# yubster4525/image_compression_2

Measured on AMD Instinct MI355X. Metric: images/sec encode+decode 256px, higher is better.
Workload: dtype f16 (synthesis) / split-bf16 (encoder); 1 GPU; batch=32 256x256 encode+8bit quantize+decode, SG3-T-256 generator; global_batch=32, per_gpu_batch=32, resolution=256, generator=stylegan3-t-256 (random init), encoder=HVAE_VGG_Encoder(img_resolution=1024), quantization_bits=8, parallelism=dp1 (batch-sharded, RCCL metric all_reduce)

## Files before the change

image_compression_2_amd/csrc/conv_common.h:

```cpp
#pragma once
#include "common.h"

namespace ic2 {

typedef __attribute__((ext_vector_type(8))) __bf16 bf16x8;
typedef __attribute__((ext_vector_type(8))) _Float16 f16x8;
typedef __attribute__((ext_vector_type(4))) float f32x4;

template <bool F16>
__device__ __forceinline__ f32x4 mfma32(bf16x8 a, bf16x8 b, f32x4 c) {
  if constexpr (F16)
    return __builtin_amdgcn_mfma_f32_16x16x32_f16(__builtin_bit_cast(f16x8, a), __builtin_bit_cast(f16x8, b), c, 0, 0, 0);
  else
    return __builtin_amdgcn_mfma_f32_16x16x32_bf16(a, b, c, 0, 0, 0);
}
__host__ __device__ inline bool is16(int dtype) { return dtype == IC2_BF16 || dtype == IC2_F16; }

struct IgemmArgs {
  const void* x;
  const void* w;
  void* y;
  const float* oscale;
  const float* bias;
  float* ws;
  int n, h, w_, cin_p, cout_p, cout_valid, kh, kw, pad, ho, wo;
  int M;
  int K;
  int nq;
  int tiles_o;
  int nblocks;
  int group;
  int korder;
  int o_base;
  int tile_base;
  int act;
  float slope, act_gain, clamp, out_mul;
  int out_layout, out_dtype;
  double* gn_part;
  int gn_groups, gn_c;
  const float* in_gn;
  float in_slope;
  int x_pix, x_hb32;
  int x_img, x_plane;
  int wx_twp, wx_th, wx_ns, wx_hp, wx_nh, wx_tx, wx_ty;
  int out_ieee;
};
__device__ __forceinline__ int ig_xb32(const IgemmArgs& a, int b) { return b >= a.x_hb32 ? b - a.x_hb32 : b; }
__device__ __forceinline__ uint32_t ig_halo_off(const IgemmArgs& a, int nn, int iy, int ix, int chunk) {
  return (uint32_t)((nn * a.x_img + (iy * a.w_ + ix) * a.x_pix) * 2 + (chunk >> 1) * a.x_plane + (chunk & 1) * 16);
}
inline void ig_set_input_layout(IgemmArgs& a, bool blocked) {
  if (blocked) a.x_pix = 16;
  a.x_img = blocked ? a.cin_p * a.h * a.w_ : a.x_pix * a.h * a.w_;
  a.x_plane = blocked ? a.h * a.w_ * 32 : 32;
}

__device__ __forceinline__ float4 ig_load_oscale(const IgemmArgs& a, int nn, int ob) {
  return a.oscale && ob < a.cout_p ? *reinterpret_cast<const float4*>(a.oscale + (int64_t)nn * a.cout_p + ob)
                                   : make_float4(1.f, 1.f, 1.f, 1.f);
}
__device__ __forceinline__ float4 ig_load_bias(const IgemmArgs& a, int ob) {
  return a.bias && ob < a.cout_p ? *reinterpret_cast<const float4*>(a.bias + ob) : make_float4(0.f, 0.f, 0.f, 0.f);
}
__device__ __forceinline__ void ig_preloads_done() { __builtin_amdgcn_s_waitcnt(0x0F70); }

__device__ __forceinline__ void ig_store4v(const IgemmArgs& a, int p, int nn, int pix, int ob, const float (&acc)[4],
                                           float4 sc, float4 bi, float (*vout)[4] = nullptr) {
  const float scv[4] = {sc.x, sc.y, sc.z, sc.w}, biv[4] = {bi.x, bi.y, bi.z, bi.w};
  float v[4];
#pragma unroll
  for (int r = 0; r < 4; ++r) {
    float t = acc[r] * scv[r] + biv[r];
    if (a.act) t = lrelu_gain_clamp(t, a.slope, a.act_gain, a.clamp);
    v[r] = t * a.out_mul;
  }
  if (vout != nullptr) {
#pragma unroll
    for (int r = 0; r < 4; ++r) (*vout)[r] = v[r];
  }
  if (a.out_layout != IC2_LAYOUT_NCHW) {
    const int64_t e = a.out_layout == IC2_LAYOUT_NHWC
                          ? (int64_t)p * a.cout_p + ob
                          : (((int64_t)nn * (a.cout_p >> 4) + (ob >> 4)) * ((int64_t)a.ho * a.wo) + pix) * 16 + (ob & 15);
    if (a.out_dtype == IC2_BF16) {
      uint2 pk;
      pk.x = (uint32_t)f2bf(v[0]) | ((uint32_t)f2bf(v[1]) << 16);
      pk.y = (uint32_t)f2bf(v[2]) | ((uint32_t)f2bf(v[3]) << 16);
      *reinterpret_cast<uint2*>(reinterpret_cast<bf16_t*>(a.y) + e) = pk;
    } else if (a.out_dtype == IC2_F16) {
      typedef _Float16 h2 __attribute__((ext_vector_type(2)));
      float s_[4];
#pragma unroll
      for (int r = 0; r < 4; ++r) s_[r] = a.out_ieee ? v[r] : __builtin_amdgcn_fmed3f(v[r], -65504.f, 65504.f);
      const h2 q0 = h2{(_Float16)s_[0], (_Float16)s_[1]}, q1 = h2{(_Float16)s_[2], (_Float16)s_[3]};
      if (vout != nullptr) {
        (*vout)[0] = (float)q0.x; (*vout)[1] = (float)q0.y; (*vout)[2] = (float)q1.x; (*vout)[3] = (float)q1.y;
      }
      uint2 pk;
      pk.x = __builtin_bit_cast(uint32_t, q0);
      pk.y = __builtin_bit_cast(uint32_t, q1);
      *reinterpret_cast<uint2*>(reinterpret_cast<uint16_t*>(a.y) + e) = pk;
    } else {
      *reinterpret_cast<float4*>(reinterpret_cast<float*>(a.y) + e) = make_float4(v[0], v[1], v[2], v[3]);
    }
  } else {
    float* yo = reinterpret_cast<float*>(a.y);
    const int hw = a.ho * a.wo;
#pragma unroll
    for (int r = 0; r < 4; ++r)
      if (ob + r < a.cout_valid) yo[((int64_t)nn * a.cout_valid + ob + r) * hw + pix] = v[r];
  }
}
__device__ __forceinline__ void ig_store4(const IgemmArgs& a, int p, int nn, int pix, int ob, const float (&acc)[4]) {
  ig_store4v(a, p, nn, pix, ob, acc, ig_load_oscale(a, nn, ob), ig_load_bias(a, ob));
}

__device__ __forceinline__ int xcd_remap(int b, int nblocks) {
  const int xcd = b & 7, loc = b >> 3;
  const int q8 = nblocks >> 3, r8 = nblocks & 7;
  return (xcd < r8 ? xcd * (q8 + 1) : r8 * (q8 + 1) + (xcd - r8) * q8) + loc;
}

template <int I, int J>
__device__ __forceinline__ void ig_epilogue(const IgemmArgs& a, const f32x4 (&acc)[I][J], int obase, int pbase, int fr,
                                            int fh) {
  const int hw = a.ho * a.wo;
  if (gridDim.y > 1) {
#pragma unroll
    for (int j = 0; j < J; ++j) {
      const int p = pbase + j * 16 + fr;
      if (p >= a.M) continue;
#pragma unroll
      for (int i = 0; i < I; ++i) {
        const int ob = obase + i * 16 + 4 * fh;
        if (ob < a.cout_p) *reinterpret_cast<f32x4*>(a.ws + ((int64_t)blockIdx.y * a.M + p) * a.cout_p + ob) = acc[i][j];
      }
    }
    return;
  }
  float4 bi[I];
#pragma unroll
  for (int i = 0; i < I; ++i) bi[i] = ig_load_bias(a, obase + i * 16 + 4 * fh);
#pragma unroll
  for (int j = 0; j < J; ++j) {
    const int p = pbase + j * 16 + fr;
    const int pc = p < a.M ? p : a.M - 1;
    const int nn = pc / hw;
    const int pix = pc - nn * hw;
    float4 sc[I];
#pragma unroll
    for (int i = 0; i < I; ++i) sc[i] = ig_load_oscale(a, nn, obase + i * 16 + 4 * fh);
    ig_preloads_done();
    if (p >= a.M) continue;
#pragma unroll
    for (int i = 0; i < I; ++i) {
      const int ob = obase + i * 16 + 4 * fh;
      if (ob >= a.cout_p) continue;
      const float v[4] = {acc[i][j][0], acc[i][j][1], acc[i][j][2], acc[i][j][3]};
      ig_store4v(a, p, nn, pix, ob, v, sc[i], bi[i]);
    }
  }
}

__device__ __forceinline__ void tile_coords(int logical, int tiles_o, int tiles_p, int group, int& o_tile,
                                            int& p_tile) {
  const int per = group * tiles_o;
  const int gi = logical / per;
  const int rem = logical - gi * per;
  const int gsz = min(group, tiles_p - gi * group);
  o_tile = rem / gsz;
  p_tile = gi * group + (rem - o_tile * gsz);
}

constexpr uint32_t kOob = 0x7ffffff0u;
constexpr int kRsrcWord3 = 0x00020000;

}
```

image_compression_2_amd/csrc/wino.hip:

```cpp
#include "conv_common.h"

namespace ic2 {

constexpr int WX_BO = 128, WX_NW = 8, WX_NS = 3;
constexpr int WX_SLAB = 4 * WX_BO * 64;
constexpr int WX_HROWS = 384, WX_HALO = WX_HROWS * 64;
constexpr int WX_HPW = WX_HROWS / 16 / WX_NW;
constexpr int WX_SLACK = 8 * 1024;
constexpr int WX_LDS = WX_NS * WX_SLAB + 2 * WX_HALO + WX_SLACK;
static_assert(WX_LDS <= 160 * 1024, "LDS");

typedef __attribute__((ext_vector_type(4))) uint32_t wx_u4;
__device__ __forceinline__ f16x8 wx_sub(f16x8 a, f16x8 b) {
  const wx_u4 x = __builtin_bit_cast(wx_u4, a), y = __builtin_bit_cast(wx_u4, b);
  wx_u4 r;
#pragma unroll
  for (int i = 0; i < 4; ++i) asm("v_pk_add_f16 %0, %1, %2 neg_lo:[0,1] neg_hi:[0,1]" : "=v"(r[i]) : "v"(x[i]), "v"(y[i]));
  return __builtin_bit_cast(f16x8, r);
}
__device__ __forceinline__ f16x8 wx_add(f16x8 a, f16x8 b) {
  const wx_u4 x = __builtin_bit_cast(wx_u4, a), y = __builtin_bit_cast(wx_u4, b);
  wx_u4 r;
#pragma unroll
  for (int i = 0; i < 4; ++i) asm("v_pk_add_f16 %0, %1, %2" : "=v"(r[i]) : "v"(x[i]), "v"(y[i]));
  return __builtin_bit_cast(f16x8, r);
}

__device__ __forceinline__ int wx_off(int row, int chunk) { return row * 64 + ((chunk ^ (((row >> 2) & 1) << 1)) << 4); }
__device__ __forceinline__ int wx_hoff(int line, int hp, int idx, int chunk) {
  return (line * hp + idx) * 64 + ((chunk ^ (((idx >> 2) & 1) << 1)) << 4);
}

#ifndef IC2_WX_ABL
#define IC2_WX_ABL 0
#endif
#ifndef IC2_WX_STAMP
#define IC2_WX_STAMP 0
#endif
#ifndef IC2_WX_SCHED
#define IC2_WX_SCHED 0
#endif
#ifndef IC2_WX_PRIO
#define IC2_WX_PRIO 0
#endif

__global__ void __launch_bounds__(512, 1) wino_fx_f16_kernel(IgemmArgs a) {
  __shared__ __attribute__((aligned(16))) char lds[WX_LDS];
  char* const wsl = lds;
  char* const hal = lds + WX_NS * WX_SLAB;
  const int tid = threadIdx.x;
  const int lane = tid & 63;
  const int wid = __builtin_amdgcn_readfirstlane(tid >> 6);
  const int half = wid >> 2;
  const int pg = wid & 3;
  const int fr = lane & 15, fh = lane >> 4;

  const int logical = xcd_remap(blockIdx.x, a.nblocks);
  const int per_group = a.group * (a.nblocks / a.tiles_o);
  const int gi = logical / per_group, grem = logical - gi * per_group;
  const int o_tile = gi * a.group + grem % a.group;
  int pt = grem / a.group;
  const int tx = pt % a.wx_tx;
  pt /= a.wx_tx;
  const int ty = pt % a.wx_ty;
  const int nn = pt / a.wx_ty;
  const int o0 = o_tile * WX_BO;
  const int twp = a.wx_twp, hp = a.wx_hp;
  const int oy0 = ty * a.wx_th, px0 = tx * twp;

  const char* __restrict__ xg = reinterpret_cast<const char*>(a.x);
  const char* __restrict__ ug = reinterpret_cast<const char*>(a.w);
  const int lrow = lane >> 2, pch = lane & 3;

  uint32_t w_off[2][2];
#pragma unroll
  for (int h = 0; h < 2; ++h)
#pragma unroll
    for (int k = 0; k < 2; ++k) {
      const int row = (wid + WX_NW * k) * 16 + lrow;
      const int nu = row >> 6, ol = h * 64 + (row & 63), o = o0 + ol;
      w_off[h][k] =
          o < a.cout_p ? (uint32_t)(((ol * 12 + nu) * a.cin_p) * 2 + ((pch ^ (((row >> 2) & 1) << 1)) << 4)) : kOob;
    }
  const char* const ug0 = ug + (int64_t)o0 * 12 * a.cin_p * 2;
  uint32_t h_off[WX_HPW];
#pragma unroll
  for (int k = 0; k < WX_HPW; ++k) {
    const int l = (wid + WX_NW * k) * 16 + lrow;
    const int line = l / hp, idx = l - line * hp;
    const int iy = oy0 - a.pad + (line >> 1), ix = 2 * px0 - a.pad + 2 * idx + (line & 1);
    const bool ok = l < a.wx_nh && (unsigned)iy < (unsigned)a.h && (unsigned)ix < (unsigned)a.w_;
    h_off[k] = ok ? ig_halo_off(a, nn, iy, ix, pch ^ (((idx >> 2) & 1) << 1)) : kOob;
  }
  int boff[2][3];
  const int ns = a.wx_ns;
#pragma unroll
  for (int jb = 0; jb < 2; ++jb) {
    const int b = pg * 2 + jb;
    const int rr = min(b / ns, a.wx_th - 1), t = (b % ns) * 16 + fr;
#pragma unroll
    for (int m = 0; m < 3; ++m) {
      const int j = half + m;
      boff[jb][m] = wx_hoff(rr * 2 + (j & 1), hp, t + (j >> 1), fh);
    }
  }
  const int ky_step = 2 * hp * 64;
  const int aoff = wx_off(fr, fh) + half * 2 * 64 * 64;
  const int CB = a.cin_p >> 5;
  const int x_cb = 2 * a.x_plane;

  auto issue_hs = [&](int cb, int j) {
    const __amdgpu_buffer_rsrc_t rs = __builtin_amdgcn_make_buffer_rsrc(
        (void*)(ug0 + ((int64_t)(4 * (j >> 1)) * a.cin_p + cb * 32) * 2), 0, cb < CB ? kOob : 0, kRsrcWord3);
    char* dst = wsl + j * (WX_SLAB / 2);
#pragma unroll
    for (int k = 0; k < 2; ++k)
      __builtin_amdgcn_raw_ptr_buffer_load_lds(
          rs, (__attribute__((address_space(3))) void*)(dst + (wid + WX_NW * k) * 1024), 16, w_off[j & 1][k], 0, 0, 0);
  };
  auto issue_hp = [&](int cb, int k) {
    const __amdgpu_buffer_rsrc_t rs =
        __builtin_amdgcn_make_buffer_rsrc((void*)(xg + (int64_t)cb * x_cb), 0, cb < CB ? kOob : 0, kRsrcWord3);
    __builtin_amdgcn_raw_ptr_buffer_load_lds(
        rs, (__attribute__((address_space(3))) void*)(hal + (cb & 1) * WX_HALO + (wid + WX_NW * k) * 1024), 16,
        h_off[k], 0, 0, 0);
  };

  f32x4 acc[2][8][2];
#pragma unroll
  for (int nl = 0; nl < 2; ++nl)
#pragma unroll
    for (int i = 0; i < 8; ++i)
#pragma unroll
      for (int jb = 0; jb < 2; ++jb) acc[nl][i][jb] = f32x4{0.f, 0.f, 0.f, 0.f};

  f16x8 d[2][3];
  f16x8 v[2][2];
  auto read_d = [&](const char* hl) {
#pragma unroll
    for (int jb = 0; jb < 2; ++jb)
#pragma unroll
      for (int m = 0; m < 3; ++m) d[jb][m] = *reinterpret_cast<const f16x8*>(hl + boff[jb][m]);
  };
  auto make_v = [&]() {
    if (half == 0) {
#pragma unroll
      for (int jb = 0; jb < 2; ++jb) {
        v[0][jb] = wx_sub(d[jb][0], d[jb][2]);
        v[1][jb] = wx_add(d[jb][1], d[jb][2]);
      }
    } else {
#pragma unroll
      for (int jb = 0; jb < 2; ++jb) {
        v[0][jb] = wx_sub(d[jb][1], d[jb][0]);
        v[1][jb] = wx_sub(d[jb][0], d[jb][2]);
      }
    }
  };

  issue_hp(0, 0);
  issue_hp(0, 1);
  issue_hp(0, 2);
#pragma unroll
  for (int j = 0; j < 5; ++j) issue_hs(0, j);
  issue_hp(1, 0);
  if constexpr (IC2_WX_SCHED == 2) {
    asm volatile("s_waitcnt vmcnt(5)" ::: "memory");
  } else {
    issue_hp(1, 1);
    asm volatile("s_waitcnt vmcnt(6)" ::: "memory");
  }
  __builtin_amdgcn_s_barrier();
  read_d(hal);
  bf16x8 af[2][4];
  auto read_a = [&](const char* wl, int nl) {
#pragma unroll
    for (int i = 0; i < 4; ++i) af[nl][i] = *reinterpret_cast<const bf16x8*>(wl + (nl * 64 + i * 16) * 64);
  };
  if (half == 1) __builtin_amdgcn_s_barrier();
  __builtin_amdgcn_sched_barrier(0);

  uint64_t st[7] = {0, 0, 0, 0, 0, 0, 0};
  uint64_t t_prev = 0, t_loop = 0;
  auto stamp = [&](int k) {
    if constexpr (IC2_WX_STAMP) {
      const uint64_t t = __builtin_amdgcn_s_memtime();
      st[k] += t - t_prev;
      t_prev = t;
    }
  };
  if constexpr (IC2_WX_STAMP) t_loop = t_prev = __builtin_amdgcn_s_memtime();
  for (int cb = 0; cb < CB; ++cb) {
    const char* hb_cur = hal + (cb & 1) * WX_HALO;
    const char* hb_nxt = hal + ((cb + 1) & 1) * WX_HALO;
#pragma unroll
    for (int j = 0; j < 6; ++j) {
      const int ky = j >> 1, hx = j & 1;
      const char* wl = wsl + j * (WX_SLAB / 2) + aoff;
      auto r_dma = [&]() {
        if (!(IC2_WX_ABL & 1) || cb == 0) issue_hs(cb + (j + 5) / 6, (j + 5) % 6);
        if constexpr (IC2_WX_SCHED == 2) {
          if (j == 0) issue_hp(cb + 1, 1);
          if (j == 1) issue_hp(cb + 1, 2);
          if (j == 5) issue_hp(cb + 2, 0);
        } else {
          if (j == 0) issue_hp(cb + 1, 2);
          if (j >= 4) issue_hp(cb + 2, j - 4);
        }
      };
      if constexpr (IC2_WX_PRIO == 2) __builtin_amdgcn_s_setprio(1);
      if constexpr (IC2_WX_SCHED >= 1) r_dma();
      if (hx == 0) make_v();
      read_a(wl, 0);
      read_a(wl, 1);
      if (hx == 1 && IC2_WX_SCHED < 2) {
        if constexpr (!(IC2_WX_ABL & 4)) read_d(ky < 2 ? hb_cur + (ky + 1) * ky_step : hb_nxt);
      }
      if constexpr (IC2_WX_STAMP) {
        __builtin_amdgcn_sched_barrier(0);
        stamp(0);
      }
      if constexpr (IC2_WX_SCHED == 0) r_dma();
      __builtin_amdgcn_sched_barrier(0);
      stamp(1);
      if constexpr (!(IC2_WX_ABL & 16)) {
        if constexpr (IC2_WX_SCHED == 2) {
          if (j == 1) asm volatile("s_waitcnt vmcnt(9)" ::: "memory");
          if (j == 0 || j == 2) asm volatile("s_waitcnt vmcnt(8)" ::: "memory");
          if (j == 3 || j == 5) asm volatile("s_waitcnt vmcnt(7)" ::: "memory");
          if (j == 4) asm volatile("s_waitcnt vmcnt(6)" ::: "memory");
        } else {
          if (j == 0) asm volatile("s_waitcnt vmcnt(9)" ::: "memory");
          if (j == 1 || j == 5) asm volatile("s_waitcnt vmcnt(8)" ::: "memory");
          if (j == 2 || j == 4) asm volatile("s_waitcnt vmcnt(7)" ::: "memory");
          if (j == 3) asm volatile("s_waitcnt vmcnt(6)" ::: "memory");
        }
      }
      stamp(2);
      if constexpr (!(IC2_WX_ABL & 2)) __builtin_amdgcn_s_barrier();
      asm volatile("s_waitcnt lgkmcnt(0)" ::: "memory");
      __builtin_amdgcn_sched_barrier(0);
      stamp(3);
      if constexpr (IC2_WX_PRIO == 0) __builtin_amdgcn_s_setprio(1);
      if constexpr (IC2_WX_PRIO == 2) __builtin_amdgcn_s_setprio(0);
#pragma unroll
      for (int nl = 0; nl < 2; ++nl) {
#pragma unroll
        for (int i = 0; i < 4; ++i)
#pragma unroll
          for (int jb = 0; jb < 2; ++jb) {
            if constexpr (IC2_WX_ABL & 8) asm volatile("" ::"v"(af[nl][i]), "v"(v[nl][jb]));
            else
              acc[nl][4 * hx + i][jb] =
                  mfma32<true>(af[nl][i], __builtin_bit_cast(bf16x8, v[nl][jb]), acc[nl][4 * hx + i][jb]);
          }
        if (IC2_WX_SCHED == 2 && hx == 1 && nl == 0) {
          __builtin_amdgcn_sched_barrier(0);
          if constexpr (!(IC2_WX_ABL & 4)) read_d(ky < 2 ? hb_cur + (ky + 1) * ky_step : hb_nxt);
          __builtin_amdgcn_sched_barrier(0);
        }
      }
      if constexpr (IC2_WX_PRIO == 0) __builtin_amdgcn_s_setprio(0);
      __builtin_amdgcn_sched_barrier(0);
      if constexpr (IC2_WX_STAMP) {
        asm volatile("s_waitcnt lgkmcnt(0)" ::: "memory");
      }
      stamp(4);
      if constexpr (!(IC2_WX_ABL & 2)) __builtin_amdgcn_s_barrier();
      __builtin_amdgcn_sched_barrier(0);
      stamp(5);
    }
  }
  if constexpr (IC2_WX_STAMP) {
    st[6] = __builtin_amdgcn_s_memtime() - t_loop;
    if (lane == 0) {
      uint64_t* o = reinterpret_cast<uint64_t*>(a.ws) + ((int64_t)blockIdx.x * 8 + wid) * 8;
#pragma unroll
      for (int k = 0; k < 7; ++k) o[k] = st[k];
    }
  }
  if (half == 0) __builtin_amdgcn_s_barrier();
  asm volatile("s_waitcnt vmcnt(0)" ::: "memory");
  __syncthreads();

  float2* ex = reinterpret_cast<float2*>(lds);
  auto exi = [&](int giver, int i, int jb, int e) { return ((((pg * 2 + giver) * 4 + i) * 2 + jb) * 4 + e) * 64 + lane; };
  if (half == 0) {
#pragma unroll
    for (int i = 0; i < 4; ++i)
#pragma unroll
      for (int jb = 0; jb < 2; ++jb)
#pragma unroll
        for (int e = 0; e < 4; ++e) {
          const float p0 = acc[0][4 + i][jb][e], p1 = acc[1][4 + i][jb][e];
          ex[exi(0, i, jb, e)] = make_float2(p0 + p1, p1);
        }
  } else {
#pragma unroll
    for (int i = 0; i < 4; ++i)
#pragma unroll
      for (int jb = 0; jb < 2; ++jb)
#pragma unroll
        for (int e = 0; e < 4; ++e) {
          const float p0 = acc[0][i][jb][e], p1 = acc[1][i][jb][e];
          ex[exi(1, i, jb, e)] = make_float2(p0, p0 + p1);
        }
  }
  __syncthreads();
  const int hw = a.ho * a.wo;
  float4 sc[4], bi[4];
#pragma unroll
  for (int i = 0; i < 4; ++i) {
    const int ob = o0 + (4 * half + i) * 16 + 4 * fh;
    sc[i] = ig_load_oscale(a, nn, ob);
    bi[i] = ig_load_bias(a, ob);
  }
  ig_preloads_done();
#pragma unroll
  for (int jb = 0; jb < 2; ++jb) {
    const int b = pg * 2 + jb;
    const int r = b / ns, t = (b % ns) * 16 + fr;
    if (r >= a.wx_th || t >= twp) continue;
    const int oy = oy0 + r, ox = 2 * (px0 + t);
    if (oy >= a.ho || ox >= a.wo) continue;
    const int pix = oy * a.wo + ox;
#pragma unroll
    for (int i = 0; i < 4; ++i) {
      const int ob = o0 + (4 * half + i) * 16 + 4 * fh;
      if (ob >= a.cout_p) continue;
      float y0[4], y1[4];
      if (half == 0) {
#pragma unroll
        for (int e = 0; e < 4; ++e) {
          const float2 q = ex[exi(1, i, jb, e)];
          const float p0 = acc[0][i][jb][e], p1 = acc[1][i][jb][e];
          y0[e] = p0 + p1 + q.x;
          y1[e] = p1 - q.y;
        }
      } else {
#pragma unroll
        for (int e = 0; e < 4; ++e) {
          const float2 q = ex[exi(0, i, jb, e)];
          const float p0 = acc[0][4 + i][jb][e], p1 = acc[1][4 + i][jb][e];
          y0[e] = q.x + p0;
          y1[e] = q.y - (p0 + p1);
        }
      }
      ig_store4v(a, nn * hw + pix, nn, pix, ob, y0, sc[i], bi[i]);
      if (ox + 1 < a.wo) ig_store4v(a, nn * hw + pix + 1, nn, pix + 1, ob, y1, sc[i], bi[i]);
    }
  }
}

__global__ void __launch_bounds__(256) pack_wino_kernel(const float* __restrict__ w, int cout, int cin, int cout_p,
                                                        int cin_p, int prenorm, float gscale,
                                                        _Float16* __restrict__ out) {
  const int o = blockIdx.x;
  __shared__ float red[256];
  float scale = gscale;
  if (o < cout && prenorm) {
    float s = 0.f;
    for (int i = threadIdx.x; i < cin * 9; i += 256) {
      const float v = w[(int64_t)o * cin * 9 + i];
      s += v * v;
    }
    red[threadIdx.x] = s;
    __syncthreads();
    for (int off = 128; off > 0; off >>= 1) {
      if (threadIdx.x < off) red[threadIdx.x] += red[threadIdx.x + off];
      __syncthreads();
    }
    scale *= rsqrtf(red[0] / (float)(cin * 9));
  }
  for (int e = threadIdx.x; e < 3 * cin_p; e += 256) {
    const int ky = e / cin_p, c = e - ky * cin_p;
    float g0 = 0.f, g1 = 0.f, g2 = 0.f;
    if (o < cout && c < cin) {
      const float* p = w + ((int64_t)o * cin + c) * 9 + ky * 3;
      g0 = p[0] * scale;
      g1 = p[1] * scale;
      g2 = p[2] * scale;
    }
    const float u[4] = {g0, 0.5f * (g0 + g1 + g2), 0.5f * (g0 - g1 + g2), g2};
    _Float16* row = out + ((int64_t)o * 3 + ky) * 4 * cin_p + c;
#pragma unroll
    for (int nu = 0; nu < 4; ++nu) row[nu * cin_p] = (_Float16)__builtin_amdgcn_fmed3f(u[nu], -65504.f, 65504.f);
  }
}

struct WxTile {
  int twp, th, ns, hp, nh, tx, ty, to;
  int64_t blocks;
};
static WxTile wx_tile(int n, int ho, int wo, int cout_p) {
  static const int force_twp = knob("IC2_WINO_TWP", 0), force_th = knob("IC2_WINO_TH", 0);
  const int pairs = (wo + 1) / 2;
  WxTile best{};
  int64_t best_rounds = -1;
  for (int ns = 1; ns <= 8; ns *= 2)
    for (int th = 1; th * ns <= 8; ++th) {
      if (force_th && th != force_th) continue;
      for (int twp = 1; twp <= 16 * ns; ++twp) {
        if (force_twp && twp != force_twp) continue;
        const int hp = twp + 1, nh = (th + 2) * 2 * hp;
        if (nh > WX_HROWS) break;
        WxTile t;
        t.twp = twp; t.th = th; t.ns = ns; t.hp = hp; t.nh = nh;
        t.tx = (int)ceil_div(pairs, twp);
        t.ty = (int)ceil_div(ho, th);
        t.to = (int)ceil_div(cout_p, WX_BO);
        t.blocks = (int64_t)n * t.tx * t.ty * t.to;
        const int64_t rounds = ceil_div(t.blocks, 256);
        const bool full = twp % 16 == 0, best_full = best.twp % 16 == 0;
        if (best_rounds < 0 || rounds < best_rounds ||
            (rounds == best_rounds && (t.blocks < best.blocks || (t.blocks == best.blocks && full && !best_full)))) {
          best = t;
          best_rounds = rounds;
        }
      }
    }
  return best;
}

static int wx_chunk_n(int n, int h, int w_, int cin_p) {
  const int64_t per_img = (int64_t)h * w_ * cin_p * 2;
  if ((int64_t)n * per_img < (int64_t)kOob || per_img >= (int64_t)kOob) return n;
  const int64_t c = ((int64_t)kOob - 1) / per_img;
  return (int)ceil_div(n, ceil_div(n, c));
}

static void* g_wx_stamp = nullptr;
static int64_t g_wx_stamp_bytes = 0;

}

using namespace ic2;

extern "C" int ic2_conv_wino_stamps(void* buf, int64_t bytes) {
  IC2_CHECK_ARG(IC2_WX_STAMP, "conv_wino_stamps: not a stamp build (IC2_WX_STAMP)");
  g_wx_stamp = buf;
  g_wx_stamp_bytes = bytes;
  return IC2_OK;
}

extern "C" int ic2_pack_weight_wino(const float* w, int cout, int cin, int cout_p, int cin_p, int prenorm,
                                    float scale, void* u_out, int dtype, void* stream) {
  IC2_CHECK_ARG(w && u_out && cout > 0 && cin > 0 && cout_p >= cout && cin_p >= cin, "pack_weight_wino: bad arguments");
  IC2_CHECK_ARG(dtype == IC2_F16, "pack_weight_wino: only f16 U (dtype %d)", dtype);
  hipLaunchKernelGGL(pack_wino_kernel, dim3(cout_p), dim3(256), 0, as_stream(stream), w, cout, cin, cout_p, cin_p,
                     prenorm, scale, (_Float16*)u_out);
  IC2_CHECK_LAUNCH("pack_weight_wino");
  return IC2_OK;
}

extern "C" int ic2_conv_wino_preferred(int dtype, int n, int h, int w_, int cin_p, int cout_p, int kh, int kw,
                                       int pad) {
  static const int mode = knob("IC2_WINO", 1);
  const int ho = h + 2 * pad - kh + 1, wo = w_ + 2 * pad - kw + 1;
  const bool legal = dtype == IC2_F16 && kh == 3 && kw == 3 && n > 0 && ho > 0 && wo > 0 && cin_p % 32 == 0 &&
                     cout_p % 32 == 0 && (int64_t)cout_p * 12 * cin_p * 2 < (int64_t)kOob;
  if (!legal || mode == 0) return 0;
  if (mode == 2) return 1;
  return cin_p >= 256 && cout_p >= 256 && ho >= 50 && wo >= 50;
}

extern "C" const char* ic2_conv_wino_plan(int n, int h, int w_, int cin_p, int cout_p, int pad) {
  const int ho = h + 2 * pad - 2, wo = w_ + 2 * pad - 2;
  if (n <= 0 || ho <= 0 || wo <= 0 || cin_p <= 0 || cin_p % 32 || cout_p <= 0 || cout_p % 32) return "invalid";
  const WxTile t = wx_tile(wx_chunk_n(n, h, w_, cin_p), ho, wo, cout_p);
  static thread_local char buf[64];
  snprintf(buf, sizeof(buf), "wino_fx_o128_p%dx%d_f16", t.twp, t.th);
  return buf;
}

extern "C" int ic2_conv_wino(const void* x, const void* u, void* y, int dtype, int out_dtype, int n, int h, int w_,
                             int cin_p, int cout_p, int cout_valid, int pad, int ho, int wo, const float* oscale,
                             const float* bias, int act, float slope, float act_gain, float clamp, float out_mul,
                             int out_layout, void* stream) {
  IC2_CHECK_ARG(x && u && y, "conv_wino: null pointer");
  IC2_CHECK_ARG(dtype == IC2_F16, "conv_wino: f16 operands only (dtype %d)", dtype);
  const int act_flags = act, in_layout = IC2_ACT_IN_LAYOUT_OF(act_flags);
  act = IC2_ACT_OF(act_flags);
  IC2_CHECK_ARG(in_layout == IC2_LAYOUT_NHWC || in_layout == IC2_LAYOUT_NHWC16, "conv_wino: bad input layout %d",
                in_layout);
  const bool in_blocked = in_layout == IC2_LAYOUT_NHWC16;
  IC2_CHECK_ARG(out_dtype == IC2_F32 || out_dtype == IC2_BF16 ||
                    ((out_dtype == IC2_F16 || out_dtype == IC2_F16_IEEE) && out_layout != IC2_LAYOUT_NCHW),
                "conv_wino: bad out dtype %d", out_dtype);
  IC2_CHECK_ARG(cin_p > 0 && cin_p % 32 == 0 && cout_p > 0 && cout_p % 32 == 0,
                "conv_wino: channel strides must be positive multiples of 32 (cin_p=%d cout_p=%d)", cin_p, cout_p);
  IC2_CHECK_ARG(n > 0 && h > 0 && w_ > 0 && pad >= 0, "conv_wino: bad geometry");
  IC2_CHECK_ARG(ho == h + 2 * pad - 2 && wo == w_ + 2 * pad - 2 && ho > 0 && wo > 0,
                "conv_wino: output size %dx%d does not match input %dx%d, k=3x3, pad=%d", ho, wo, h, w_, pad);
  IC2_CHECK_ARG(out_layout == IC2_LAYOUT_NHWC || out_layout == IC2_LAYOUT_NHWC16 ||
                    (out_layout == IC2_LAYOUT_NCHW && out_dtype == IC2_F32 && cout_valid > 0 && cout_valid <= cout_p),
                "conv_wino: NCHW output needs f32 and 0 < cout_valid <= cout_p (layout %d)", out_layout);
  IC2_CHECK_ARG(((uintptr_t)oscale | (uintptr_t)bias) % 16 == 0, "conv_wino: oscale/bias must be 16-byte aligned");
  IC2_CHECK_ARG((int64_t)cout_p * 12 * cin_p * 2 < (int64_t)kOob, "conv_wino: weights too large");
  const int nc = wx_chunk_n(n, h, w_, cin_p);
  if (nc < n) {
    const int64_t x_img = (int64_t)h * w_ * cin_p * 2;
    const int64_t y_img = out_layout == IC2_LAYOUT_NCHW ? (int64_t)cout_valid * ho * wo * 4
                                                        : (int64_t)ho * wo * cout_p * (out_dtype == IC2_F32 ? 4 : 2);
    for (int n0 = 0; n0 < n; n0 += nc) {
      const int nn = n - n0 < nc ? n - n0 : nc;
      const int rc = ic2_conv_wino(reinterpret_cast<const char*>(x) + n0 * x_img, u,
                                   reinterpret_cast<char*>(y) + n0 * y_img, dtype, out_dtype, nn, h, w_, cin_p, cout_p,
                                   cout_valid, pad, ho, wo, oscale ? oscale + (int64_t)n0 * cout_p : nullptr, bias,
                                   act_flags, slope, act_gain, clamp, out_mul, out_layout, stream);
      if (rc != IC2_OK) return rc;
    }
    return IC2_OK;
  }
  const WxTile t = wx_tile(n, ho, wo, cout_p);
  IC2_CHECK_ARG(t.blocks > 0 && t.blocks < (1LL << 31), "conv_wino: bad tile plan");
  const int out_ieee = out_dtype == IC2_F16_IEEE;
  if (out_ieee) out_dtype = IC2_F16;
  IgemmArgs a{};
  a.x = x; a.w = u; a.y = y; a.oscale = oscale; a.bias = bias;
  a.ws = IC2_WX_STAMP && (int64_t)t.blocks * 8 * 8 * 8 <= g_wx_stamp_bytes ? reinterpret_cast<float*>(g_wx_stamp)
                                                                          : nullptr;
  IC2_CHECK_ARG(!IC2_WX_STAMP || a.ws, "conv_wino: stamp build without a large enough ic2_conv_wino_stamps buffer");
  a.n = n; a.h = h; a.w_ = w_; a.cin_p = cin_p; a.cout_p = cout_p; a.cout_valid = cout_valid;
  a.kh = 3; a.kw = 3; a.pad = pad; a.ho = ho; a.wo = wo;
  a.M = n * ho * wo; a.K = 9 * cin_p; a.nq = 3 * (cin_p / 32);
  static const int og_knob = knob("IC2_WINO_OGROUP", 1);
  int og = og_knob < 1 ? 1 : og_knob > t.to ? t.to : og_knob;
  while (t.to % og) --og;
  a.tiles_o = t.to; a.nblocks = (int)t.blocks; a.group = og; a.korder = 1; a.o_base = 0;
  a.act = act; a.slope = slope; a.act_gain = act_gain; a.clamp = clamp; a.out_mul = out_mul;
  a.out_layout = out_layout; a.out_dtype = out_dtype; a.out_ieee = out_ieee;
  a.gn_part = nullptr; a.gn_groups = 0; a.gn_c = 0; a.in_gn = nullptr; a.in_slope = 0.f;
  a.x_pix = cin_p; a.x_hb32 = 0;
  ig_set_input_layout(a, in_blocked);
  a.wx_twp = t.twp; a.wx_th = t.th; a.wx_ns = t.ns; a.wx_hp = t.hp; a.wx_nh = t.nh; a.wx_tx = t.tx; a.wx_ty = t.ty;
  hipLaunchKernelGGL(wino_fx_f16_kernel, dim3((unsigned)t.blocks), dim3(64 * WX_NW), 0, as_stream(stream), a);
  IC2_CHECK_LAUNCH("conv_wino");
  return IC2_OK;
}
```

Measured before the change: 1529 images/s.

## Add flat pixel-slot tiling mode to Winograd conv with LDS-conflict-aware tile search

Adds a 'flat' mapping for Winograd output tiles in which 16-lane slots are laid out linearly over a th×twp tile instead of per-row strips. This lets tile shapes not aligned to multiples of 16 fill slots densely. A host-side search scores candidate tiles by launch rounds, block count and a modelled LDS bank-conflict count. It picks flat tiling only when that saves a margin of rounds over the row-based scheme. Tile choices are memoized per shape, and the kernel gains a runtime branch on the flat flag.

```diff
diff --git a/image_compression_2_amd/csrc/conv_common.h b/image_compression_2_amd/csrc/conv_common.h
--- a/image_compression_2_amd/csrc/conv_common.h
+++ b/image_compression_2_amd/csrc/conv_common.h
@@ -44,6 +44,7 @@
   int x_img, x_plane;
   int wx_twp, wx_th, wx_ns, wx_hp, wx_nh, wx_tx, wx_ty;
   int out_ieee;
+  int wx_flat;
 };
 __device__ __forceinline__ int ig_xb32(const IgemmArgs& a, int b) { return b >= a.x_hb32 ? b - a.x_hb32 : b; }
 __device__ __forceinline__ uint32_t ig_halo_off(const IgemmArgs& a, int nn, int iy, int ix, int chunk) {
diff --git a/image_compression_2_amd/csrc/wino.hip b/image_compression_2_amd/csrc/wino.hip
--- a/image_compression_2_amd/csrc/wino.hip
+++ b/image_compression_2_amd/csrc/wino.hip
@@ -29,6 +29,17 @@
 __device__ __forceinline__ int wx_off(int row, int chunk) { return row * 64 + ((chunk ^ (((row >> 2) & 1) << 1)) << 4); }
 __device__ __forceinline__ int wx_hoff(int line, int hp, int idx, int chunk) {
   return (line * hp + idx) * 64 + ((chunk ^ (((idx >> 2) & 1) << 1)) << 4);
+}
+__device__ __forceinline__ bool wx_slot(const IgemmArgs& a, int b, int fr, int& r, int& t) {
+  if (a.wx_flat) {
+    const int s = 16 * b + fr;
+    r = s / a.wx_twp;
+    t = s - r * a.wx_twp;
+    return s < a.wx_th * a.wx_twp;
+  }
+  r = b / a.wx_ns;
+  t = (b % a.wx_ns) * 16 + fr;
+  return r < a.wx_th && t < a.wx_twp;
 }
 
 #ifndef IC2_WX_ABL
@@ -93,11 +104,12 @@
     h_off[k] = ok ? ig_halo_off(a, nn, iy, ix, pch ^ (((idx >> 2) & 1) << 1)) : kOob;
   }
   int boff[2][3];
-  const int ns = a.wx_ns;
 #pragma unroll
   for (int jb = 0; jb < 2; ++jb) {
-    const int b = pg * 2 + jb;
-    const int rr = min(b / ns, a.wx_th - 1), t = (b % ns) * 16 + fr;
+    int rr, t;
+    const bool live = wx_slot(a, pg * 2 + jb, fr, rr, t);
+    if (a.wx_flat && !live) t = twp - 1;
+    rr = min(rr, a.wx_th - 1);
 #pragma unroll
     for (int m = 0; m < 3; ++m) {
       const int j = half + m;
@@ -318,9 +330,8 @@
   ig_preloads_done();
 #pragma unroll
   for (int jb = 0; jb < 2; ++jb) {
-    const int b = pg * 2 + jb;
-    const int r = b / ns, t = (b % ns) * 16 + fr;
-    if (r >= a.wx_th || t >= twp) continue;
+    int r, t;
+    if (!wx_slot(a, pg * 2 + jb, fr, r, t)) continue;
     const int oy = oy0 + r, ox = 2 * (px0 + t);
     if (oy >= a.ho || ox >= a.wo) continue;
     const int pix = oy * a.wo + ox;
@@ -389,12 +400,50 @@
 }
 
 struct WxTile {
-  int twp, th, ns, hp, nh, tx, ty, to;
+  int twp, th, ns, hp, nh, tx, ty, to, flat;
   int64_t blocks;
+  int64_t rounds() const { return ceil_div(blocks, 256); }
 };
-static WxTile wx_tile(int n, int ho, int wo, int cout_p) {
-  static const int force_twp = knob("IC2_WINO_TWP", 0), force_th = knob("IC2_WINO_TH", 0);
-  const int pairs = (wo + 1) / 2;
+static WxTile wx_make_tile(int twp, int th, int ns, int flat, int n, int ho, int wo, int cout_p) {
+  WxTile t;
+  t.twp = twp; t.th = th; t.ns = ns; t.flat = flat; t.hp = twp + 1; t.nh = (th + 2) * 2 * t.hp;
+  t.tx = (int)ceil_div((wo + 1) / 2, twp);
+  t.ty = (int)ceil_div(ho, th);
+  t.to = (int)ceil_div(cout_p, WX_BO);
+  t.blocks = (int64_t)n * t.tx * t.ty * t.to;
+  return t;
+}
+
+static int wx_flat_conflicts(int twp, int th, int pitch) {
+  const int live = th * twp;
+  int bad = 0;
+  for (int b = 0; b < 8; ++b)
+    for (int j = 0; j < 4; ++j)
+      for (int ky = 0; ky < 3; ++ky) {
+        bool conflict = false;
+        for (int g = 0; g < 2; ++g) {
+          int seen[16];
+          for (int i = 0; i < 16; ++i) seen[i] = -1;
+          for (int fh = 0; fh < 2; ++fh)
+            for (int fr = 0; fr < 16; ++fr) {
+              const bool outer = fr < 4 || fr >= 12;
+              if ((fh == g) != outer) continue;
+              const int s = 16 * b + fr < live ? 16 * b + fr : live - 1;
+              const int r = s / twp, t = s - r * twp;
+              const int idx = t + (j >> 1), row = ((r + ky) * 2 + (j & 1)) * pitch + idx;
+              const int res = (row & 3) * 4 + (fh ^ (((idx >> 2) & 1) << 1));
+              if (seen[res] >= 0 && seen[res] != row) conflict = true;
+              seen[res] = row;
+            }
+        }
+        bad += conflict;
+      }
+  return bad;
+}
+
+constexpr int WX_FLAT_MARGIN_PCT = 4;
+
+static WxTile wx_tile_rows(int n, int ho, int wo, int cout_p, int force_twp, int force_th) {
   WxTile best{};
   int64_t best_rounds = -1;
   for (int ns = 1; ns <= 8; ns *= 2)
@@ -402,15 +451,9 @@
       if (force_th && th != force_th) continue;
       for (int twp = 1; twp <= 16 * ns; ++twp) {
         if (force_twp && twp != force_twp) continue;
-        const int hp = twp + 1, nh = (th + 2) * 2 * hp;
-        if (nh > WX_HROWS) break;
-        WxTile t;
-        t.twp = twp; t.th = th; t.ns = ns; t.hp = hp; t.nh = nh;
-        t.tx = (int)ceil_div(pairs, twp);
-        t.ty = (int)ceil_div(ho, th);
-        t.to = (int)ceil_div(cout_p, WX_BO);
-        t.blocks = (int64_t)n * t.tx * t.ty * t.to;
-        const int64_t rounds = ceil_div(t.blocks, 256);
+        if ((th + 2) * 2 * (twp + 1) > WX_HROWS) break;
+        const WxTile t = wx_make_tile(twp, th, ns, 0, n, ho, wo, cout_p);
+        const int64_t rounds = t.rounds();
         const bool full = twp % 16 == 0, best_full = best.twp % 16 == 0;
         if (best_rounds < 0 || rounds < best_rounds ||
             (rounds == best_rounds && (t.blocks < best.blocks || (t.blocks == best.blocks && full && !best_full)))) {
@@ -420,6 +463,47 @@
       }
     }
   return best;
+}
+static WxTile wx_tile_flat(int n, int ho, int wo, int cout_p, int force_twp, int force_th) {
+  WxTile best{};
+  int best_conf = 0;
+  for (int th = 1; th <= 128; ++th) {
+    if (force_th && th != force_th) continue;
+    for (int twp = 1; th * twp <= 128; ++twp) {
+      if (force_twp && twp != force_twp) continue;
+      if ((th + 2) * 2 * (twp + 1) > WX_HROWS) break;
+      const WxTile t = wx_make_tile(twp, th, 0, 1, n, ho, wo, cout_p);
+      if (best.blocks > 0 && (t.rounds() > best.rounds() || (t.rounds() == best.rounds() && t.blocks > best.blocks)))
+        continue;
+      const int conf = wx_flat_conflicts(twp, th, t.hp);
+      if (best.blocks > 0 && t.rounds() == best.rounds() && t.blocks == best.blocks &&
+          (conf > best_conf || (conf == best_conf && t.nh >= best.nh)))
+        continue;
+      best = t;
+      best_conf = conf;
+    }
+  }
+  return best;
+}
+static WxTile wx_tile_search(int n, int ho, int wo, int cout_p, int mode, int force_twp, int force_th) {
+  const WxTile rows = wx_tile_rows(n, ho, wo, cout_p, force_twp, force_th);
+  if (mode == 0) return rows;
+  const WxTile flat = wx_tile_flat(n, ho, wo, cout_p, force_twp, force_th);
+  if (mode == 2 || rows.blocks == 0) return flat;
+  if (flat.blocks == 0) return rows;
+  return flat.rounds() * 100 <= rows.rounds() * (100 - WX_FLAT_MARGIN_PCT) ? flat : rows;
+}
+static WxTile wx_tile(int n, int ho, int wo, int cout_p) {
+  static const int force_twp = knob("IC2_WINO_TWP", 0), force_th = knob("IC2_WINO_TH", 0);
+  static const int mode = knob("IC2_WINO_FLAT", 1);
+  struct Memo { int n, ho, wo, cout_p; WxTile t; };
+  static thread_local Memo memo[16];
+  static thread_local int memo_n = 0;
+  for (int i = 0; i < (memo_n < 16 ? memo_n : 16); ++i)
+    if (memo[i].n == n && memo[i].ho == ho && memo[i].wo == wo && memo[i].cout_p == cout_p) return memo[i].t;
+  const WxTile t = wx_tile_search(n, ho, wo, cout_p, mode, force_twp, force_th);
+  memo[memo_n++ % 16] = Memo{n, ho, wo, cout_p, t};
+  return t;
 }
 
 static int wx_chunk_n(int n, int h, int w_, int cin_p) {
@@ -469,7 +553,7 @@
   if (n <= 0 || ho <= 0 || wo <= 0 || cin_p <= 0 || cin_p % 32 || cout_p <= 0 || cout_p % 32) return "invalid";
   const WxTile t = wx_tile(wx_chunk_n(n, h, w_, cin_p), ho, wo, cout_p);
   static thread_local char buf[64];
-  snprintf(buf, sizeof(buf), "wino_fx_o128_p%dx%d_f16", t.twp, t.th);
+  snprintf(buf, sizeof(buf), "wino_fx_o128_p%dx%d%s_f16", t.twp, t.th, t.flat ? "w" : "");
   return buf;
 }
 
@@ -534,6 +618,7 @@
   a.x_pix = cin_p; a.x_hb32 = 0;
   ig_set_input_layout(a, in_blocked);
   a.wx_twp = t.twp; a.wx_th = t.th; a.wx_ns = t.ns; a.wx_hp = t.hp; a.wx_nh = t.nh; a.wx_tx = t.tx; a.wx_ty = t.ty;
+  a.wx_flat = t.flat;
   hipLaunchKernelGGL(wino_fx_f16_kernel, dim3((unsigned)t.blocks), dim3(64 * WX_NW), 0, as_stream(stream), a);
   IC2_CHECK_LAUNCH("conv_wino");
   return IC2_OK;
```

Result: faster. 1546 images/s (median of 6 runs) (+1.2%).
